# naver/dust3r

Hardware: NVIDIA H100
Metric: image-pairs/sec (512x384, ViT-L/B+DPT) (higher is better)
Workload: dtype bf16

## Files before the change

### dust3r_b200/csrc/d3r_common.cuh

```cuda
#pragma once
#include <cuda.h>
#include <cuda_runtime.h>
#include <cuda_bf16.h>
#include <cstdint>
#include <cstdio>
#include <cstdarg>

#include "../../include/dust3r_b200.h"

namespace d3r {

void set_error(const char* fmt, ...);

#define D3R_CHECK_ARG(cond, ...)                    \
  do {                                              \
    if (!(cond)) {                                  \
      ::d3r::set_error(__VA_ARGS__);                \
      return D3R_ERR_INVALID;                       \
    }                                               \
  } while (0)

#define D3R_CUDA(expr)                                                                     \
  do {                                                                                     \
    cudaError_t _e = (expr);                                                               \
    if (_e != cudaSuccess) {                                                               \
      ::d3r::set_error("%s failed: %s (%s:%d)", #expr, cudaGetErrorString(_e), __FILE__, __LINE__); \
      return D3R_ERR_CUDA;                                                                 \
    }                                                                                      \
  } while (0)

#define D3R_LAUNCH_CHECK()                                                                 \
  do {                                                                                     \
    cudaError_t _e = cudaGetLastError();                                                   \
    if (_e != cudaSuccess) {                                                               \
      ::d3r::set_error("kernel launch failed: %s (%s:%d)", cudaGetErrorString(_e), __FILE__, __LINE__); \
      return D3R_ERR_CUDA;                                                                 \
    }                                                                                      \
  } while (0)

__device__ __forceinline__ float warp_sum(float v) {
  v += __shfl_xor_sync(0xffffffffu, v, 16);
  v += __shfl_xor_sync(0xffffffffu, v, 8);
  v += __shfl_xor_sync(0xffffffffu, v, 4);
  v += __shfl_xor_sync(0xffffffffu, v, 2);
  v += __shfl_xor_sync(0xffffffffu, v, 1);
  return v;
}

__device__ __forceinline__ uint32_t pack_bf16x2(float a, float b) {
  __nv_bfloat162 h = __floats2bfloat162_rn(a, b);
  return *reinterpret_cast<uint32_t*>(&h);
}
__device__ __forceinline__ float2 bf16x2_to_float2(uint32_t w) {
  const __nv_bfloat162 h = *reinterpret_cast<const __nv_bfloat162*>(&w);
  return make_float2(__low2float(h), __high2float(h));
}

template <class ConfIn>
__device__ __forceinline__ void postprocess_pixel(float x, float y, float z, ConfIn conf_in, float* pts3d, float* conf, long long pix,
                                                  int depth_mode, int conf_mode, float cmin, float cmax) {
  float ox = x, oy = y, oz = z;
  if (depth_mode != 0) {
    const float d = sqrtf(x * x + y * y + z * z);
    const float dc = fmaxf(d, 1e-8f);
    const float s = (depth_mode == 2) ? expm1f(d) : d * d;
    ox = x / dc * s; oy = y / dc * s; oz = z / dc * s;
  }
  float* o = pts3d + pix * 3;
  o[0] = ox; o[1] = oy; o[2] = oz;
  if (conf_mode != 0) {
    const float c = conf_in();
    float r;
    if (conf_mode == 1) r = cmin + fminf(expf(c), cmax - cmin);
    else r = (cmax - cmin) * (1.f / (1.f + expf(-c))) + cmin;
    conf[pix] = r;
  }
}

int num_sms();

int encode_tensor_map(CUtensorMap* m, const void* base, int rank, const cuuint64_t* dims, const cuuint64_t* strides_bytes,
                      const cuuint32_t* box, const char* op, CUtensorMapDataType dtype = CU_TENSOR_MAP_DATA_TYPE_BFLOAT16);

inline bool first_launch_on_this_device(unsigned long long& mask) {
  int dev = 0;
  cudaGetDevice(&dev);
  const unsigned long long bit = 1ull << (dev & 63);
  if (mask & bit) return false;
  mask |= bit;
  return true;
}

}
```

### dust3r_b200/csrc/gemm_host.cu

```cuda
#include "gemm_wgmma.cuh"
#include "gemm_host.h"
#include "prof.h"

namespace d3r {
namespace gemm {

static int pick_block_n(int N, int mode, uint32_t flags, int conv_m_tiles = 0) {
  if (flags & F_HEAD_FINAL) return 128;
  if (conv_m_tiles > 0) return (N == 256 && (conv_m_tiles + 1) / 2 >= 4 * (num_sms() / 2)) ? 256 : 128;
  if (N % 256 == 0 && pick_epi(mode, flags) != EPI_GENERIC) return 256;
  if (N % 128 == 0) return 128;
  if (N % 64 == 0) return 64;
  return (N > 128) ? 128 : 64;
}

static int g_impl = 2;
static int g_pair_min_kb = 4;
static bool use_pair(int bn, int num_kb) { return bn >= 128 && (g_impl == 1 || (g_impl == 2 && num_kb >= g_pair_min_kb)); }

static int g_store = 1;
static int g_conv_store = 1;

static int grid_for(bool pair, int m_tiles, int n_tiles) {
  if (pair) {
    const int items = ((m_tiles + 1) / 2) * n_tiles;
    const int max_clusters = num_sms() / 2;
    return 2 * (items < max_clusters ? items : max_clusters);
  }
  const int items = m_tiles * n_tiles;
  return items < num_sms() ? items : num_sms();
}

static const char* prof_tag(const Params& p, int bn, bool pair) {
  return (p.mode == 1) ? ((p.flags & F_HEAD_FINAL) ? (pair ? "conv3x3_head_tail_2cta" : "conv3x3_head_tail")
                                                   : (pair ? "conv3x3_wgmma_2cta" : "conv3x3_wgmma"))
                       : (bn == 256 ? (pair ? "gemm_wgmma_2cta_bn256" : "gemm_wgmma_bn256")
                                    : (pair ? "gemm_wgmma_2cta_bn128" : (bn == 128 ? "gemm_wgmma_bn128" : "gemm_wgmma_bn64")));
}

template <int BN, int EPI, bool PAIR, bool TMA_STORE = false>
static int launch(const CUtensorMap& ta, const CUtensorMap& tb, const CUtensorMap& to, const Params& p, int m_tiles, int n_tiles,
                  cudaStream_t st) {
  constexpr int kSmem = Cfg<BN, TMA_STORE>::kSmemBytes;
  static unsigned long long attr_devices = 0;
  if (first_launch_on_this_device(attr_devices))
    D3R_CUDA(cudaFuncSetAttribute(gemm_kernel<BN, EPI, PAIR, TMA_STORE>, cudaFuncAttributeMaxDynamicSharedMemorySize, kSmem));
  const int grid = grid_for(PAIR, m_tiles, n_tiles);
  char detail[96];
  snprintf(detail, sizeof(detail), "M=%d N=%d K=%d flags=0x%x mode=%d epi=%d", p.M, p.N, p.K, (unsigned)p.flags, p.mode, EPI);
  prof::Scope scope(prof_tag(p, BN, PAIR), st, 2.0 * double(p.M) * double(p.N) * double(p.K), 0.0, 1, detail);
  D3R_CUDA(pdl::launch_clustered(gemm_kernel<BN, EPI, PAIR, TMA_STORE>, dim3(grid), dim3(kNumThreads), size_t(kSmem), st, PAIR ? 2 : 1,
                                 ta, tb, to, p));
  D3R_LAUNCH_CHECK();
  return D3R_OK;
}

template <int BN, bool PAIR>
static int launch_conv(const CUtensorMap& ta, const CUtensorMap& tb, const CUtensorMap& to, const ConvMaps& cm, const Params& p,
                       int m_tiles, int n_tiles, cudaStream_t st) {
  constexpr int kSmem = Cfg<BN, true>::kSmemBytes;
  static unsigned long long attr_devices = 0;
  if (first_launch_on_this_device(attr_devices))
    D3R_CUDA(cudaFuncSetAttribute(conv_kernel<BN, PAIR>, cudaFuncAttributeMaxDynamicSharedMemorySize, kSmem));
  const int grid = grid_for(PAIR, m_tiles, n_tiles);
  char detail[96];
  snprintf(detail, sizeof(detail), "M=%d N=%d K=%d flags=0x%x mode=%d epi=%d", p.M, p.N, p.K, (unsigned)p.flags, p.mode, EPI_GENERIC);
  prof::Scope scope(prof_tag(p, BN, PAIR), st, 2.0 * double(p.M) * double(p.N) * double(p.K), 0.0, 1, detail);
  D3R_CUDA(pdl::launch_clustered(conv_kernel<BN, PAIR>, dim3(grid), dim3(kNumThreads), size_t(kSmem), st, PAIR ? 2 : 1, ta, tb, to, cm, p));
  D3R_LAUNCH_CHECK();
  return D3R_OK;
}

template <int BN, bool PAIR>
static int dispatch_epi(int epi, const CUtensorMap& ta, const CUtensorMap& tb, const CUtensorMap* to, const Params& p, int m_tiles,
                        int n_tiles, cudaStream_t st) {
  if constexpr (BN == 256) {
    if (to) {
      switch (epi) {
        case EPI_RESID: return launch<BN, EPI_RESID, PAIR, true>(ta, tb, *to, p, m_tiles, n_tiles, st);
        case EPI_ACT: return launch<BN, EPI_ACT, PAIR, true>(ta, tb, *to, p, m_tiles, n_tiles, st);
        case EPI_ROPE: return launch<BN, EPI_ROPE, PAIR, true>(ta, tb, *to, p, m_tiles, n_tiles, st);
      }
    }
  }
  switch (epi) {
    case EPI_RESID: return launch<BN, EPI_RESID, PAIR>(ta, tb, tb, p, m_tiles, n_tiles, st);
    case EPI_ACT: return launch<BN, EPI_ACT, PAIR>(ta, tb, tb, p, m_tiles, n_tiles, st);
    case EPI_ROPE: return launch<BN, EPI_ROPE, PAIR>(ta, tb, tb, p, m_tiles, n_tiles, st);
  }
  if constexpr (BN == 128) return launch<128, EPI_GENERIC, PAIR>(ta, tb, tb, p, m_tiles, n_tiles, st);
  set_error("no BLOCK_N %d kernel for the generic epilogue", BN);
  return D3R_ERR_INVALID;
}

static int dispatch(int bn, const CUtensorMap& ta, const CUtensorMap& tb, const CUtensorMap* to, const Params& p, int m_tiles,
                    cudaStream_t st) {
  const int n_tiles = (p.N + bn - 1) / bn;
  const int epi = (bn >= 128) ? pick_epi(p.mode, p.flags) : EPI_GENERIC;
  const bool pair = use_pair(bn, p.num_kb);
  switch (bn) {
    case 256: return pair ? dispatch_epi<256, true>(epi, ta, tb, to, p, m_tiles, n_tiles, st) : dispatch_epi<256, false>(epi, ta, tb, to, p, m_tiles, n_tiles, st);
    case 128: return pair ? dispatch_epi<128, true>(epi, ta, tb, nullptr, p, m_tiles, n_tiles, st) : dispatch_epi<128, false>(epi, ta, tb, nullptr, p, m_tiles, n_tiles, st);
    case 64: return launch<64, EPI_GENERIC, false>(ta, tb, tb, p, m_tiles, n_tiles, st);
  }
  set_error("unsupported BLOCK_N %d", bn);
  return D3R_ERR_INVALID;
}

static int make_tmap_b(CUtensorMap* m, const void* B, int N, int taps, int Kc, int bn, int num_kb, const char* op) {
  cuuint64_t dims[3] = {(cuuint64_t)Kc, (cuuint64_t)taps, (cuuint64_t)N};
  cuuint64_t str[2] = {(cuuint64_t)Kc * 2, (cuuint64_t)taps * Kc * 2};
  cuuint32_t box[3] = {(cuuint32_t)BLOCK_K, 1, (cuuint32_t)(use_pair(bn, num_kb) ? bn / 2 : bn)};
  return encode_tensor_map(m, B, 3, dims, str, box, op);
}

int gemm_bf16(const void* A, long long lda, const void* B, Params p, cudaStream_t st) {
  D3R_CHECK_ARG(A && B, "gemm: null operand");
  D3R_CHECK_ARG(p.M > 0 && p.N > 0 && p.K > 0, "gemm: bad shape %d %d %d", p.M, p.N, p.K);
  D3R_CHECK_ARG(p.N % 32 == 0, "gemm: N=%d must be a multiple of 32", p.N);
  D3R_CHECK_ARG(p.K % 8 == 0 && lda % 8 == 0, "gemm: K=%d / lda=%lld must be multiples of 8 (16-byte TMA strides)", p.K, lda);
  D3R_CHECK_ARG((reinterpret_cast<uintptr_t>(A) & 15) == 0 && (reinterpret_cast<uintptr_t>(B) & 15) == 0, "gemm: operands must be 16-byte aligned");
// ... 17 lines not shown
                      (reinterpret_cast<uintptr_t>(p.out) & 15) == 0;
  if (staged) {
    cuuint64_t dims[2] = {(cuuint64_t)p.N, (cuuint64_t)p.M};
    cuuint64_t str[1] = {(cuuint64_t)row_bytes};
    cuuint32_t box[2] = {(cuuint32_t)(f32 ? 32 : 64), 64};
    rc = encode_tensor_map(&to, p.out, 2, dims, str, box, "gemm output", f32 ? CU_TENSOR_MAP_DATA_TYPE_FLOAT32 : CU_TENSOR_MAP_DATA_TYPE_BFLOAT16);
    if (rc) return rc;
  }
  return dispatch(bn, ta, tb, staged ? &to : nullptr, p, (p.M + BLOCK_M - 1) / BLOCK_M, st);
}

static int make_tmap_conv_io(CUtensorMap* m, const void* base, int B, int H, int W, int C, int tile_w, const char* op) {
  const int bw = tile_w < 64 ? tile_w : 64;
  cuuint64_t dims[4] = {(cuuint64_t)C, (cuuint64_t)W, (cuuint64_t)H, (cuuint64_t)B};
  cuuint64_t str[3] = {(cuuint64_t)C * 2, (cuuint64_t)W * C * 2, (cuuint64_t)H * W * C * 2};
  cuuint32_t box[4] = {64, (cuuint32_t)bw, (cuuint32_t)(64 / bw), 1};
  return encode_tensor_map(m, base, 4, dims, str, box, op);
}

static bool aligned16(const void* ptr) { return (reinterpret_cast<uintptr_t>(ptr) & 15) == 0; }

int conv3x3_bf16(const void* x_nhwc, const void* w_packed, int B, int H, int W, int Cin, int Cout, Params p, cudaStream_t st) {
  D3R_CHECK_ARG(x_nhwc && w_packed, "conv3x3: null operand");
  D3R_CHECK_ARG(Cin % 8 == 0 && Cout % 32 == 0, "conv3x3: Cin=%d must be a multiple of 8 and Cout=%d of 32", Cin, Cout);
  p.mode = 1;
  p.M = B * H * W;
  p.N = Cout;
  p.cin_blocks = (Cin + BLOCK_K - 1) / BLOCK_K;
  p.K = 9 * Cin;
  p.num_kb = 9 * p.cin_blocks;
  p.cB = B; p.cH = H; p.cW = W;
  int tw = 16;
  while (tw < W && tw < 128) tw *= 2;
  p.tile_w = tw;
  p.tile_h = BLOCK_M / tw;
  p.tiles_x = (W + p.tile_w - 1) / p.tile_w;
  p.tiles_y = (H + p.tile_h - 1) / p.tile_h;
  p.ldo = Cout;
  const int m_tiles = B * p.tiles_x * p.tiles_y;
  const bool staged = g_conv_store == 1 && (Cout == 256 || Cout == 128) && (p.flags & ~EpiMask<EPI_CONV>::value) == 0 &&
                      aligned16(p.out) && (!(p.flags & F_OUT2_RELU) || aligned16(p.out2)) && (!(p.flags & F_ADD0) || aligned16(p.add0)) &&
                      (!(p.flags & F_ADD1) || aligned16(p.add1));
  const int bn = pick_block_n(p.N, p.mode, p.flags, staged ? m_tiles : 0);
  CUtensorMap ta, tb;
  {
    cuuint64_t dims[4] = {(cuuint64_t)Cin, (cuuint64_t)W, (cuuint64_t)H, (cuuint64_t)B};
    cuuint64_t str[3] = {(cuuint64_t)Cin * 2, (cuuint64_t)W * Cin * 2, (cuuint64_t)H * W * Cin * 2};
    cuuint32_t box[4] = {(cuuint32_t)BLOCK_K, (cuuint32_t)p.tile_w, (cuuint32_t)p.tile_h, 1};
    int rc = encode_tensor_map(&ta, x_nhwc, 4, dims, str, box, "conv3x3");
    if (rc) return rc;
  }
  int rc = make_tmap_b(&tb, w_packed, Cout, 9, Cin, bn, p.num_kb, "conv3x3");
  if (rc) return rc;
  if (!staged) return dispatch(bn, ta, tb, nullptr, p, m_tiles, st);
  CUtensorMap to;
  ConvMaps cm;
  rc = make_tmap_conv_io(&to, p.out, B, H, W, Cout, p.tile_w, "conv3x3 output");
  if (rc) return rc;
  cm.out2 = cm.add0 = cm.add1 = to;
  const struct { uint32_t flag; const void* base; CUtensorMap* map; const char* op; } io[3] = {
      {F_OUT2_RELU, p.out2, &cm.out2, "conv3x3 out2"}, {F_ADD0, p.add0, &cm.add0, "conv3x3 add0"}, {F_ADD1, p.add1, &cm.add1, "conv3x3 add1"}};
  for (const auto& t : io) {
    if (!(p.flags & t.flag)) continue;
    rc = make_tmap_conv_io(t.map, t.base, B, H, W, Cout, p.tile_w, t.op);
    if (rc) return rc;
  }
  const int n_tiles = Cout / bn;
  const bool pair = use_pair(bn, p.num_kb);
  if (bn == 256) return pair ? launch_conv<256, true>(ta, tb, to, cm, p, m_tiles, n_tiles, st) : launch_conv<256, false>(ta, tb, to, cm, p, m_tiles, n_tiles, st);
  return pair ? launch_conv<128, true>(ta, tb, to, cm, p, m_tiles, n_tiles, st) : launch_conv<128, false>(ta, tb, to, cm, p, m_tiles, n_tiles, st);
}

int conv_transpose_bf16(const void* x_nhwc, const void* w_packed, void* out, const float* bias, int B, int h, int w, int Cin, int Cout,
                        int k, cudaStream_t st) {
  D3R_CHECK_ARG(x_nhwc && w_packed && out, "conv_transpose: null buffer");
  D3R_CHECK_ARG(B > 0 && h > 0 && w > 0 && Cin > 0 && Cout > 0 && k > 0, "conv_transpose: bad shape B=%d h=%d w=%d Cin=%d Cout=%d k=%d", B,
                h, w, Cin, Cout, k);
  D3R_CHECK_ARG(Cin % 8 == 0, "conv_transpose: Cin=%d must be a multiple of 8", Cin);
  D3R_CHECK_ARG(Cout % 2 == 0 && (k * k * Cout) % 32 == 0, "conv_transpose: Cout=%d must be even and k*k*Cout=%d a multiple of 32", Cout,
                k * k * Cout);
  Params p{};
  p.M = B * h * w; p.N = k * k * Cout; p.K = Cin;
  p.flags = F_CONVT | (bias ? F_BIAS : 0);
  p.out = out; p.bias = bias; p.ldo = 0;
  p.tk = k; p.th_in = h; p.tw_in = w; p.tCout = Cout;
  return gemm_bf16(x_nhwc, Cin, w_packed, p, st);
}

int conv3x3_head_tail(const void* x_nhwc, const void* w_packed, const float* bias, const float* w4, const float* b4, float* pts3d,
                      float* conf, int B, int H, int W, int depth_mode, int conf_mode, float conf_min, float conf_max, cudaStream_t st) {
  D3R_CHECK_ARG(x_nhwc && w_packed && w4 && b4 && pts3d, "conv3x3_head_tail: null buffer");
  D3R_CHECK_ARG(B > 0 && H > 0 && W > 0, "conv3x3_head_tail: bad shape B=%d H=%d W=%d", B, H, W);
  D3R_CHECK_ARG(depth_mode >= 0 && depth_mode <= 2, "conv3x3_head_tail: depth_mode %d out of range", depth_mode);
  D3R_CHECK_ARG(conf_mode >= 0 && conf_mode <= 2, "conv3x3_head_tail: conf_mode %d out of range", conf_mode);
  D3R_CHECK_ARG(conf_mode == 0 || conf, "conv3x3_head_tail: conf_mode %d without a conf buffer", conf_mode);
  Params p{};
  p.flags = F_HEAD_FINAL | (bias ? F_BIAS : 0);
  p.bias = bias;
  p.w4 = w4; p.b4 = b4;
  p.pts3d = pts3d; p.conf = conf;
  p.depth_mode = depth_mode; p.conf_mode = conf_mode;
  p.conf_min = conf_min; p.conf_max = conf_max;
  return conv3x3_bf16(x_nhwc, w_packed, B, H, W, 128, 128, p, st);
}

}
// ... 46 lines not shown
```

### dust3r_b200/csrc/gemm_wgmma.cuh

```cuda
#pragma once
#include "d3r_common.cuh"
#include "sm90_ptx.cuh"
#include "pdl.cuh"

namespace d3r {
namespace gemm {

constexpr int BLOCK_M = 128;
constexpr int BLOCK_K = 64;
constexpr int WGMMA_K = 16;
constexpr int kNumThreads = 384;
constexpr int kConsumerWarps = 8;

enum : uint32_t {
  F_BIAS = 1u << 0,
  F_GELU = 1u << 1,
  F_RELU = 1u << 2,
  F_OUT_F32 = 1u << 3,
  F_RESID_INPLACE = 1u << 4,
  F_ADD0 = 1u << 5,
  F_ADD1 = 1u << 6,
  F_OUT2_RELU = 1u << 7,
  F_ROPE = 1u << 8,
  F_CONVT = 1u << 9,
  F_HEAD_FINAL = 1u << 10,
  F_OUT2_BF16 = 1u << 11,
};

struct Params {
  int M, N, K;
  int num_kb;
  int mode;
  uint32_t flags;
  void* out;
  void* out2;
  const void* add0;
  const void* add1;
  const float* bias;
  long long ldo;
  const float* rope_cos;
  const float* rope_sin;
  int rope_cols, tokens_per_img, grid_w;
  int cB, cH, cW, cin_blocks, tile_w, tile_h, tiles_x, tiles_y;
  int tk, th_in, tw_in, tCout;
  const float* w4;
  const float* b4;
  float* pts3d;
  float* conf;
  int depth_mode;
  int conf_mode;
  float conf_min, conf_max;
};

enum : int { EPI_GENERIC = 0, EPI_RESID = 1, EPI_ACT = 2, EPI_ROPE = 3, EPI_CONV = 4 };
template <int EPI> struct EpiMask { static constexpr uint32_t value = 0xFFFFFFFFu; };
template <> struct EpiMask<EPI_RESID> { static constexpr uint32_t value = F_BIAS | F_RESID_INPLACE; };
template <> struct EpiMask<EPI_ACT> { static constexpr uint32_t value = F_BIAS | F_GELU | F_RELU; };
template <> struct EpiMask<EPI_ROPE> { static constexpr uint32_t value = F_BIAS | F_ROPE; };
template <> struct EpiMask<EPI_CONV> { static constexpr uint32_t value = F_BIAS | F_RELU | F_ADD0 | F_ADD1 | F_OUT2_RELU; };

struct ConvMaps {
  CUtensorMap out2, add0, add1;
};

__host__ __device__ inline int pick_epi(int mode, uint32_t flags) {
  if (mode != 0) return EPI_GENERIC;
  if ((flags & ~F_BIAS) == F_RESID_INPLACE) return EPI_RESID;
  if ((flags & ~EpiMask<EPI_ACT>::value) == 0) return EPI_ACT;
  if ((flags & ~EpiMask<EPI_ROPE>::value) == 0) return EPI_ROPE;
  return EPI_GENERIC;
}

template <int BLOCK_N, bool TMA_STORE = false>
struct Cfg {
  static constexpr int kStageA = BLOCK_M * BLOCK_K * 2;
  static constexpr int kStageB = BLOCK_N * BLOCK_K * 2;
  static constexpr int kStages = (BLOCK_N == 256) ? 4 : (BLOCK_N == 128) ? 6 : 8;
  static constexpr int kRing = kStages * (kStageA + kStageB);
  static constexpr int kOutBuf = 64 * 128;
  static constexpr int kStaging = TMA_STORE ? 2 * 2 * kOutBuf : 0;
  static constexpr int kSmemBytes = kRing + kStaging + 1024  + 256  + (TMA_STORE ? 0 : (4 * 128 + 16) * 4) ;
  static_assert(kSmemBytes <= 227 * 1024, "shared memory of one CTA");
};

__device__ __forceinline__ float gelu_erf(float x) {
  constexpr float kU = 0.84932180028801904f;
  constexpr float kP = 0.3275911f * 0.70710678118654752f / kU;
  const float u = fabsf(x) * kU;
  const float t = ptx::rcp_approx(fmaf(kP, u, 1.f));
  float poly = fmaf(0.5f * 1.061405429f, t, 0.5f * -1.453152027f);
  poly = fmaf(poly, t, 0.5f * 1.421413741f);
  poly = fmaf(poly, t, 0.5f * -0.284496736f);
  poly = fmaf(poly, t, 0.5f * 0.254829592f);
  const float e = ptx::ex2_approx(-u * u);
  const float h = x * (poly * t * e);
  return fmaxf(x, 0.f) - fabsf(h);
}

template <int BLOCK_N, int EPI, bool PAIR, bool TMA_STORE>
__device__ __forceinline__ void gemm_body(const CUtensorMap& tmap_a, const CUtensorMap& tmap_b, const CUtensorMap& tmap_o,
                                          const ConvMaps* cm, const Params& p) {
  static_assert(EPI == EPI_CONV ? (TMA_STORE && (BLOCK_N == 256 || BLOCK_N == 128))
                                : (!TMA_STORE || (BLOCK_N == 256 && EPI != EPI_GENERIC)),
                "TMA-store epilogue: specialised projection epilogues on 128x256 tiles, the conv epilogue on 128x256 / 128x128");
  using C = Cfg<BLOCK_N, TMA_STORE>;
  extern __shared__ uint8_t smem_raw[];
  uint8_t* smem = reinterpret_cast<uint8_t*>((reinterpret_cast<uintptr_t>(smem_raw) + 1023) & ~uintptr_t(1023));
  uint8_t* smem_a = smem;
  uint8_t* smem_b = smem + C::kStages * C::kStageA;
  uint8_t* smem_o = smem + C::kRing;
  uint64_t* bars = reinterpret_cast<uint64_t*>(smem + C::kRing + C::kStaging);
  uint64_t* full_bar = bars;
  uint64_t* empty_bar = bars + C::kStages;
  uint64_t* add_bar = bars + 2 * C::kStages;
  float* s_w4 = reinterpret_cast<float*>(reinterpret_cast<uint8_t*>(bars) + 256);

  const int warp = threadIdx.x >> 5, lane = threadIdx.x & 31;
  const uint32_t rank = PAIR ? ptx::cluster_ctarank() : 0u;
  const int n_tiles = (p.N + BLOCK_N - 1) / BLOCK_N;
  const int m_tiles = (p.mode == 1) ? p.cB * p.tiles_y * p.tiles_x : (p.M + BLOCK_M - 1) / BLOCK_M;
  const int m_groups = PAIR ? (m_tiles + 1) / 2 : m_tiles;
  const int total_items = m_groups * n_tiles;
  const int first_item = PAIR ? blockIdx.x / 2 : blockIdx.x;
  const int item_stride = PAIR ? gridDim.x / 2 : gridDim.x;

  if (threadIdx.x == 0) {
    ptx::prefetch_tmap(&tmap_a);
    ptx::prefetch_tmap(&tmap_b);
    if constexpr (TMA_STORE) ptx::prefetch_tmap(&tmap_o);
    for (int s = 0; s < C::kStages; ++s) {
      ptx::mbar_init(ptx::smem_u32(&full_bar[s]), 1);
      ptx::mbar_init(ptx::smem_u32(&empty_bar[s]), (PAIR ? 2 : 1) * kConsumerWarps);
    }
    if constexpr (EPI == EPI_CONV) {
      ptx::prefetch_tmap(&cm->out2);
      ptx::prefetch_tmap(&cm->add0);
      ptx::prefetch_tmap(&cm->add1);
      ptx::mbar_init(ptx::smem_u32(&add_bar[0]), 1);
      ptx::mbar_init(ptx::smem_u32(&add_bar[1]), 1);
    }
    ptx::fence_barrier_init();
  }
  if (!TMA_STORE && (p.flags & F_HEAD_FINAL) && threadIdx.x >= 128) {
    for (int i = threadIdx.x - 128; i < 4 * 128 + 4; i += 256) s_w4[i] = (i < 512) ? p.w4[i] : p.b4[i - 512];
  }
  __syncthreads();
  if constexpr (PAIR) ptx::cluster_sync();
  pdl::sync_with_predecessor();

  if (warp < 4) {
    ptx::setmaxnreg_dec<40>();
    if (warp == 0 && ptx::elect_one()) {
      int stage = 0;
      uint32_t phase = 0;
      for (int item = first_item; item < total_items; item += item_stride) {
        const int tn = item % n_tiles, tm = (item / n_tiles) * (PAIR ? 2 : 1) + int(rank);
        int cb = 0, cy0 = 0, cx0 = 0;
        if (p.mode == 1) {
          cb = tm / (p.tiles_y * p.tiles_x);
          const int r = tm - cb * (p.tiles_y * p.tiles_x);
          cy0 = (r / p.tiles_x) * p.tile_h;
          cx0 = (r % p.tiles_x) * p.tile_w;
        }
        for (int kb = 0; kb < p.num_kb; ++kb) {
          ptx::mbar_wait(ptx::smem_u32(&empty_bar[stage]), phase ^ 1);
          const uint32_t fb = ptx::smem_u32(&full_bar[stage]);
          ptx::mbar_arrive_expect_tx(fb, C::kStageA + C::kStageB);
          const uint32_t sa = ptx::smem_u32(smem_a + stage * C::kStageA);
          const uint32_t sb = ptx::smem_u32(smem_b + stage * C::kStageB);
          int ka, kt = 0;
          if (p.mode == 1) {
            const int tap = kb / p.cin_blocks, cblk = kb - tap * p.cin_blocks;
            const int dy = tap / 3, dx = tap - dy * 3;
            ptx::tma_load_4d(sa, &tmap_a, fb, cblk * BLOCK_K, cx0 + dx - 1, cy0 + dy - 1, cb);
            ka = cblk * BLOCK_K;
            kt = tap;
          } else {
            ptx::tma_load_2d(sa, &tmap_a, fb, kb * BLOCK_K, tm * BLOCK_M);
            ka = kb * BLOCK_K;
          }
          if constexpr (PAIR) {
            constexpr int kHalf = BLOCK_N / 2;
            ptx::tma_load_3d_mc(sb + rank * (kHalf * BLOCK_K * 2), &tmap_b, fb, ka, kt, tn * BLOCK_N + int(rank) * kHalf, 0x3);
          } else {
            ptx::tma_load_3d(sb, &tmap_b, fb, ka, kt, tn * BLOCK_N);
          }
          if (++stage == C::kStages) { stage = 0; phase ^= 1; }
        }
      }
    }
  } else {
    ptx::setmaxnreg_inc<232>();
    const int wg = (threadIdx.x >> 7) - 1;
    const int wq = warp & 3;
    const int q = lane & 3;
    const uint32_t flags = p.flags & EpiMask<EPI>::value;
    constexpr int kNB = BLOCK_N / 8;
    float acc[BLOCK_N / 2];
    int stage = 0;
    uint32_t phase = 0;
    uint32_t out_chunk = 0;
    auto release = [&](int s) {
      if (lane == 0) {
        if constexpr (PAIR) {
          ptx::mbar_arrive_cluster(ptx::smem_u32(&empty_bar[s]), 0);
          ptx::mbar_arrive_cluster(ptx::smem_u32(&empty_bar[s]), 1);
        } else {
          ptx::mbar_arrive(ptx::smem_u32(&empty_bar[s]));
        }
      }
    };
    const bool conv_issuer = EPI == EPI_CONV && (threadIdx.x & 127) == 0;
    const bool conv_two = EPI == EPI_CONV && (flags & (F_OUT2_RELU | F_ADD1)) != 0;
    const bool conv_add = EPI == EPI_CONV && (flags & (F_ADD0 | F_ADD1)) != 0;
    uint32_t add_phase = 0;
    auto conv_box = [&](int tm, int& bx, int& by, int& bb) {
      bb = tm / (p.tiles_y * p.tiles_x);
      const int r = tm - bb * (p.tiles_y * p.tiles_x);
      bx = (r % p.tiles_x) * p.tile_w + (64 * wg) % p.tile_w;
      by = (r / p.tiles_x) * p.tile_h + (64 * wg) / p.tile_w;
    };
    auto out_buf = [&](int i) { return ptx::smem_u32(smem_o + (wg * 2 + i) * C::kOutBuf); };
    auto issue_addends = [&](int tm, int ch) {
      int bx, by, bb;
      conv_box(tm, bx, by, bb);
      const uint32_t b0 = conv_two ? out_buf(0) : out_buf(out_chunk & 1);
      if (conv_two) ptx::bulk_wait_group_read<0>();
      else ptx::bulk_wait_group_read<1>();
      const uint32_t bar = ptx::smem_u32(&add_bar[wg]);
      ptx::mbar_arrive_expect_tx(bar, uint32_t(C::kOutBuf) * (((flags & F_ADD0) ? 1u : 0u) + ((flags & F_ADD1) ? 1u : 0u)));
      if (flags & F_ADD0) ptx::tma_load_4d(b0, &cm->add0, bar, ch, bx, by, bb);
      if (flags & F_ADD1) ptx::tma_load_4d(out_buf(1), &cm->add1, bar, ch, bx, by, bb);
    };
    for (int item = first_item; item < total_items; item += item_stride) {
      const int tn = item % n_tiles, tm = (item / n_tiles) * (PAIR ? 2 : 1) + int(rank);
      if constexpr (EPI == EPI_CONV) {
        if (conv_add && conv_issuer) issue_addends(tm, tn * BLOCK_N);
      }
      int prev = -1;
      for (int kb = 0; kb < p.num_kb; ++kb) {
        ptx::mbar_wait(ptx::smem_u32(&full_bar[stage]), phase);
        const uint64_t da = ptx::desc_kmajor_sw128(ptx::smem_u32(smem_a + stage * C::kStageA + wg * 64 * 128));
        const uint64_t db = ptx::desc_kmajor_sw128(ptx::smem_u32(smem_b + stage * C::kStageB));
        ptx::wgmma_fence();
#pragma unroll
        for (int k = 0; k < BLOCK_K / WGMMA_K; ++k) {
          if constexpr (BLOCK_N == 256) ptx::wgmma_m64n256k16_ss(acc, da + uint64_t(2 * k), db + uint64_t(2 * k), (kb | k) != 0 ? 1u : 0u);
          else if constexpr (BLOCK_N == 128) ptx::wgmma_m64n128k16_ss(acc, da + uint64_t(2 * k), db + uint64_t(2 * k), (kb | k) != 0 ? 1u : 0u);
          else ptx::wgmma_m64n64k16_ss(acc, da + uint64_t(2 * k), db + uint64_t(2 * k), (kb | k) != 0 ? 1u : 0u);
        }
        ptx::wgmma_commit();
        ptx::wgmma_wait<1>();
        if (prev >= 0) release(prev);
        prev = stage;
        if (++stage == C::kStages) { stage = 0; phase ^= 1; }
      }
      ptx::wgmma_wait<0>();
      ptx::reg_fence(acc);
      release(prev);

      bool valid[2];
      long long row_off[2];
      int tok[2] = {0, 0};
      long long pix[2] = {0, 0};
      int ct_b[2] = {0, 0}, ct_iy[2] = {0, 0}, ct_ix[2] = {0, 0};
#pragma unroll
      for (int h = 0; h < 2; ++h) {
        const int row_in_tile = wg * 64 + wq * 16 + (lane >> 2) + 8 * h;
        if (p.mode == 1) {
          const int cb = tm / (p.tiles_y * p.tiles_x);
          const int r = tm - cb * (p.tiles_y * p.tiles_x);
          const int y = (r / p.tiles_x) * p.tile_h + row_in_tile / p.tile_w;
          const int x = (r % p.tiles_x) * p.tile_w + row_in_tile % p.tile_w;
          valid[h] = (tm < m_tiles) && (y < p.cH) && (x < p.cW);
          pix[h] = (long long)(cb * p.cH + y) * p.cW + x;
          row_off[h] = pix[h] * p.ldo;
        } else {
          const int row = tm * BLOCK_M + row_in_tile;
          valid[h] = row < p.M;
          row_off[h] = (long long)row * p.ldo;
          if (flags & F_ROPE) tok[h] = row % p.tokens_per_img;
          if (flags & F_CONVT) {
            ct_b[h] = row / (p.th_in * p.tw_in);
            const int r = row - ct_b[h] * (p.th_in * p.tw_in);
            ct_iy[h] = r / p.tw_in;
            ct_ix[h] = r - ct_iy[h] * p.tw_in;
// ... 167 lines not shown
          if (flags & F_CONVT) {
            const int kk = col / p.tCout, co = col - kk * p.tCout;
            const int ky = kk / p.tk, kx = kk - ky * p.tk;
            off = ((long long)(ct_b[h] * p.th_in * p.tk + ct_iy[h] * p.tk + ky) * (p.tw_in * p.tk) + ct_ix[h] * p.tk + kx) * p.tCout + co;
          } else {
            off = row_off[h] + col;
          }
          if (flags & F_ADD0) {
            const float2 a = bf16x2_to_float2(__ldg(reinterpret_cast<const unsigned int*>(reinterpret_cast<const __nv_bfloat16*>(p.add0) + off)));
            v0 += a.x; v1 += a.y;
          }
          if (flags & F_ADD1) {
            const float2 a = bf16x2_to_float2(__ldg(reinterpret_cast<const unsigned int*>(reinterpret_cast<const __nv_bfloat16*>(p.add1) + off)));
            v0 += a.x; v1 += a.y;
          }
          if (flags & F_RELU) { v0 = fmaxf(v0, 0.f); v1 = fmaxf(v1, 0.f); }
          if (flags & (F_OUT_F32 | F_RESID_INPLACE)) {
            float2* o = reinterpret_cast<float2*>(reinterpret_cast<float*>(p.out) + off);
            if (flags & F_RESID_INPLACE) {
              const float2 r = *o;
              v0 += r.x; v1 += r.y;
            }
            *o = make_float2(v0, v1);
            if (flags & F_OUT2_BF16) *reinterpret_cast<uint32_t*>(reinterpret_cast<__nv_bfloat16*>(p.out2) + off) = pack_bf16x2(v0, v1);
          } else {
            *reinterpret_cast<uint32_t*>(reinterpret_cast<__nv_bfloat16*>(p.out) + off) = pack_bf16x2(v0, v1);
            if (flags & F_OUT2_RELU)
              *reinterpret_cast<uint32_t*>(reinterpret_cast<__nv_bfloat16*>(p.out2) + off) = pack_bf16x2(fmaxf(v0, 0.f), fmaxf(v1, 0.f));
          }
        }
      }
    }
    if constexpr (TMA_STORE) {
      if ((threadIdx.x & 127) == 0) ptx::bulk_wait_group<0>();
    }
  }
  if constexpr (PAIR) ptx::cluster_sync();
}

template <int BLOCK_N, int EPI, bool PAIR, bool TMA_STORE>
__global__ void __launch_bounds__(kNumThreads, 1)
gemm_kernel(const __grid_constant__ CUtensorMap tmap_a, const __grid_constant__ CUtensorMap tmap_b,
            const __grid_constant__ CUtensorMap tmap_o, const Params p) {
  gemm_body<BLOCK_N, EPI, PAIR, TMA_STORE>(tmap_a, tmap_b, tmap_o, nullptr, p);
}

template <int BLOCK_N, bool PAIR>
__global__ void __launch_bounds__(kNumThreads, 1)
conv_kernel(const __grid_constant__ CUtensorMap tmap_a, const __grid_constant__ CUtensorMap tmap_b,
            const __grid_constant__ CUtensorMap tmap_o, const __grid_constant__ ConvMaps cm, const Params p) {
  gemm_body<BLOCK_N, EPI_CONV, PAIR, true>(tmap_a, tmap_b, tmap_o, &cm, p);
}

}
}
```

### dust3r_b200/csrc/sm90_ptx.cuh

```cuda
#pragma once
#include <cuda.h>
#include <cuda_runtime.h>
#include <cuda_bf16.h>
#include <cstdint>

namespace d3r {
namespace ptx {

__device__ __forceinline__ uint32_t smem_u32(const void* p) { return static_cast<uint32_t>(__cvta_generic_to_shared(p)); }

__device__ __forceinline__ bool elect_one() {
  uint32_t pred = 0;
  asm volatile(
      "{\n"
      ".reg .b32 %%rx;\n"
      ".reg .pred %%px;\n"
      "elect.sync %%rx|%%px, %1;\n"
      "@%%px mov.s32 %0, 1;\n"
      "}\n"
      : "+r"(pred)
      : "r"(0xffffffffu));
  return pred != 0;
}

// ... 51 lines not shown

__device__ __forceinline__ void prefetch_tmap(const void* tmap) {
  asm volatile("prefetch.tensormap [%0];" ::"l"(reinterpret_cast<uint64_t>(tmap)) : "memory");
}
__device__ __forceinline__ void tma_load_2d(uint32_t dst, const void* tmap, uint32_t bar, int c0, int c1) {
  asm volatile(
      "cp.async.bulk.tensor.2d.shared::cluster.global.mbarrier::complete_tx::bytes [%0], [%1, {%3, %4}], [%2];"
      ::"r"(dst), "l"(reinterpret_cast<uint64_t>(tmap)), "r"(bar), "r"(c0), "r"(c1)
      : "memory");
}
__device__ __forceinline__ void tma_load_3d(uint32_t dst, const void* tmap, uint32_t bar, int c0, int c1, int c2) {
  asm volatile(
      "cp.async.bulk.tensor.3d.shared::cluster.global.mbarrier::complete_tx::bytes [%0], [%1, {%3, %4, %5}], [%2];"
      ::"r"(dst), "l"(reinterpret_cast<uint64_t>(tmap)), "r"(bar), "r"(c0), "r"(c1), "r"(c2)
      : "memory");
}
__device__ __forceinline__ void tma_load_4d(uint32_t dst, const void* tmap, uint32_t bar, int c0, int c1, int c2, int c3) {
  asm volatile(
      "cp.async.bulk.tensor.4d.shared::cluster.global.mbarrier::complete_tx::bytes [%0], [%1, {%3, %4, %5, %6}], [%2];"
      ::"r"(dst), "l"(reinterpret_cast<uint64_t>(tmap)), "r"(bar), "r"(c0), "r"(c1), "r"(c2), "r"(c3)
      : "memory");
}
__device__ __forceinline__ void tma_load_3d_mc(uint32_t dst, const void* tmap, uint32_t bar, int c0, int c1, int c2, uint16_t mask) {
  asm volatile(
      "cp.async.bulk.tensor.3d.shared::cluster.global.mbarrier::complete_tx::bytes.multicast::cluster [%0], [%1, {%3, %4, %5}], [%2], %6;"
      ::"r"(dst), "l"(reinterpret_cast<uint64_t>(tmap)), "r"(bar), "r"(c0), "r"(c1), "r"(c2), "h"(mask)
      : "memory");
}

__device__ __forceinline__ void tma_store_2d(const void* tmap, uint32_t src, int c0, int c1) {
  asm volatile("cp.async.bulk.tensor.2d.global.shared::cta.tile.bulk_group [%0, {%2, %3}], [%1];"
               ::"l"(reinterpret_cast<uint64_t>(tmap)), "r"(src), "r"(c0), "r"(c1) : "memory");
}
__device__ __forceinline__ void tma_store_4d(const void* tmap, uint32_t src, int c0, int c1, int c2, int c3) {
  asm volatile("cp.async.bulk.tensor.4d.global.shared::cta.tile.bulk_group [%0, {%2, %3, %4, %5}], [%1];"
               ::"l"(reinterpret_cast<uint64_t>(tmap)), "r"(src), "r"(c0), "r"(c1), "r"(c2), "r"(c3) : "memory");
}
__device__ __forceinline__ void tma_reduce_add_2d(const void* tmap, uint32_t src, int c0, int c1) {
  asm volatile("cp.reduce.async.bulk.tensor.2d.global.shared::cta.add.tile.bulk_group [%0, {%2, %3}], [%1];"
               ::"l"(reinterpret_cast<uint64_t>(tmap)), "r"(src), "r"(c0), "r"(c1) : "memory");
}
__device__ __forceinline__ void bulk_commit_group() { asm volatile("cp.async.bulk.commit_group;" ::: "memory"); }
template <int N> __device__ __forceinline__ void bulk_wait_group_read() { asm volatile("cp.async.bulk.wait_group.read %0;" ::"n"(N) : "memory"); }
template <int N> __device__ __forceinline__ void bulk_wait_group() { asm volatile("cp.async.bulk.wait_group %0;" ::"n"(N) : "memory"); }
__device__ __forceinline__ void st_shared_b32(uint32_t addr, uint32_t v) { asm volatile("st.shared.b32 [%0], %1;" ::"r"(addr), "r"(v) : "memory"); }
__device__ __forceinline__ uint32_t ld_shared_b32(uint32_t addr) {
  uint32_t v;
  asm volatile("ld.shared.b32 %0, [%1];" : "=r"(v) : "r"(addr) : "memory");
  return v;
}
__device__ __forceinline__ void st_shared_v2_f32(uint32_t addr, float a, float b) {
  asm volatile("st.shared.v2.f32 [%0], {%1, %2};" ::"r"(addr), "f"(a), "f"(b) : "memory");
}
__device__ __forceinline__ void named_bar_sync(uint32_t id, uint32_t count) { asm volatile("bar.sync %0, %1;" ::"r"(id), "r"(count) : "memory"); }

__device__ __forceinline__ uint32_t cluster_ctarank() {
  uint32_t r;
  asm volatile("mov.u32 %0, %%cluster_ctarank;" : "=r"(r));
  return r;
}
__device__ __forceinline__ void cluster_sync() {
  asm volatile("barrier.cluster.arrive.release.aligned;\nbarrier.cluster.wait.acquire.aligned;" ::: "memory");
}
__device__ __forceinline__ void mbar_arrive_cluster(uint32_t bar, uint32_t rank) {
  asm volatile(
      "{\n"
      ".reg .b32 raddr;\n"
      "mapa.shared::cluster.u32 raddr, %0, %1;\n"
      "mbarrier.arrive.shared::cluster.b64 _, [raddr];\n"
      "}\n" ::"r"(bar), "r"(rank) : "memory");
}

__device__ __forceinline__ float ex2_approx(float x) { float y; asm("ex2.approx.ftz.f32 %0, %1;" : "=f"(y) : "f"(x)); return y; }
__device__ __forceinline__ float rcp_approx(float x) { float y; asm("rcp.approx.ftz.f32 %0, %1;" : "=f"(y) : "f"(x)); return y; }
__device__ __forceinline__ float rsqrt_approx(float x) { float y; asm("rsqrt.approx.ftz.f32 %0, %1;" : "=f"(y) : "f"(x)); return y; }
__device__ __forceinline__ float sqrt_approx(float x) { float y; asm("sqrt.approx.ftz.f32 %0, %1;" : "=f"(y) : "f"(x)); return y; }

template <int N> __device__ __forceinline__ void setmaxnreg_dec() { asm volatile("setmaxnreg.dec.sync.aligned.u32 %0;" ::"n"(N)); }
template <int N> __device__ __forceinline__ void setmaxnreg_inc() { asm volatile("setmaxnreg.inc.sync.aligned.u32 %0;" ::"n"(N)); }

__device__ __forceinline__ void wgmma_fence() { asm volatile("wgmma.fence.sync.aligned;" ::: "memory"); }
__device__ __forceinline__ void wgmma_commit() { asm volatile("wgmma.commit_group.sync.aligned;" ::: "memory"); }
template <int N> __device__ __forceinline__ void wgmma_wait() { asm volatile("wgmma.wait_group.sync.aligned %0;" ::"n"(N) : "memory"); }
template <int N> __device__ __forceinline__ void reg_fence(float (&d)[N]) {
#pragma unroll
  for (int i = 0; i < N; ++i) asm volatile("" : "+f"(d[i])::"memory");
}

__device__ __forceinline__ uint64_t desc_sw128(uint32_t smem_addr, uint32_t lbo_bytes) {
  uint64_t d = 0;
  d |= uint64_t((smem_addr & 0x3FFFF) >> 4);
  d |= uint64_t(lbo_bytes >> 4) << 16;
  d |= uint64_t(1024 >> 4) << 32;
  d |= uint64_t(1) << 62;
  return d;
}
__device__ __forceinline__ uint64_t desc_kmajor_sw128(uint32_t smem_addr) { return desc_sw128(smem_addr, 16); }
__device__ __forceinline__ uint64_t desc_mnmajor_sw128(uint32_t smem_addr) { return desc_sw128(smem_addr, 1024); }

__device__ __forceinline__ void wgmma_m64n64k16_ss(float* d, uint64_t desc_a, uint64_t desc_b, uint32_t accumulate) {
  asm volatile(
      "{\n"
      ".reg .pred p;\n"
      "setp.ne.b32 p, %34, 0;\n"
      "wgmma.mma_async.sync.aligned.m64n64k16.f32.bf16.bf16 "
      "{%0, %1, %2, %3, %4, %5, %6, %7, %8, %9, %10, %11, %12, %13, %14, %15, %16, %17, %18, %19, %20, %21, %22, %23, %24, %25, %26, %27, %28, %29, %30, %31}, %32, %33, p, 1, 1, 0, 0;\n"
// ... 52 lines not shown
```

Baseline: 233.2.

## Add dedicated DPT head-tail conv kernel with double-buffered accumulators and epilogue overlap

Adds a specialised head_tail_kernel for the final 3x3 conv plus the 1x1 head projection. It keeps two accumulator sets so the WGMMA mainloop of the next tile is issued while the current tile's fused ReLU/projection/postprocess epilogue runs. Bias and transposed w4 are staged in shared memory and read with vector loads. This is meant to hide epilogue latency in the head conv, at the cost of doubled accumulator registers and a larger static unrolled schedule.

After: 236.3 (median of 6 runs). +1.3%, better.

```diff
diff --git a/dust3r_b200/csrc/d3r_common.cuh b/dust3r_b200/csrc/d3r_common.cuh
--- a/dust3r_b200/csrc/d3r_common.cuh
+++ b/dust3r_b200/csrc/d3r_common.cuh
@@ -56,9 +56,7 @@
   return make_float2(__low2float(h), __high2float(h));
 }
 
-template <class ConfIn>
-__device__ __forceinline__ void postprocess_pixel(float x, float y, float z, ConfIn conf_in, float* pts3d, float* conf, long long pix,
-                                                  int depth_mode, int conf_mode, float cmin, float cmax) {
+__device__ __forceinline__ void postprocess_pts(float x, float y, float z, float* pts3d, long long pix, int depth_mode) {
   float ox = x, oy = y, oz = z;
   if (depth_mode != 0) {
     const float d = sqrtf(x * x + y * y + z * z);
@@ -68,13 +66,16 @@
   }
   float* o = pts3d + pix * 3;
   o[0] = ox; o[1] = oy; o[2] = oz;
-  if (conf_mode != 0) {
-    const float c = conf_in();
-    float r;
-    if (conf_mode == 1) r = cmin + fminf(expf(c), cmax - cmin);
-    else r = (cmax - cmin) * (1.f / (1.f + expf(-c))) + cmin;
-    conf[pix] = r;
-  }
+}
+__device__ __forceinline__ float postprocess_conf(float c, int conf_mode, float cmin, float cmax) {
+  if (conf_mode == 1) return cmin + fminf(expf(c), cmax - cmin);
+  return (cmax - cmin) * (1.f / (1.f + expf(-c))) + cmin;
+}
+template <class ConfIn>
+__device__ __forceinline__ void postprocess_pixel(float x, float y, float z, ConfIn conf_in, float* pts3d, float* conf, long long pix,
+                                                  int depth_mode, int conf_mode, float cmin, float cmax) {
+  postprocess_pts(x, y, z, pts3d, pix, depth_mode);
+  if (conf_mode != 0) conf[pix] = postprocess_conf(conf_in(), conf_mode, cmin, cmax);
 }
 
 int num_sms();
diff --git a/dust3r_b200/csrc/gemm_host.cu b/dust3r_b200/csrc/gemm_host.cu
--- a/dust3r_b200/csrc/gemm_host.cu
+++ b/dust3r_b200/csrc/gemm_host.cu
@@ -67,6 +67,21 @@
   snprintf(detail, sizeof(detail), "M=%d N=%d K=%d flags=0x%x mode=%d epi=%d", p.M, p.N, p.K, (unsigned)p.flags, p.mode, EPI_GENERIC);
   prof::Scope scope(prof_tag(p, BN, PAIR), st, 2.0 * double(p.M) * double(p.N) * double(p.K), 0.0, 1, detail);
   D3R_CUDA(pdl::launch_clustered(conv_kernel<BN, PAIR>, dim3(grid), dim3(kNumThreads), size_t(kSmem), st, PAIR ? 2 : 1, ta, tb, to, cm, p));
+  D3R_LAUNCH_CHECK();
+  return D3R_OK;
+}
+
+template <bool PAIR>
+static int launch_head(const CUtensorMap& ta, const CUtensorMap& tb, const Params& p, int m_tiles, cudaStream_t st) {
+  constexpr int kSmem = Cfg<128>::kSmemBytes;
+  static unsigned long long attr_devices = 0;
+  if (first_launch_on_this_device(attr_devices))
+    D3R_CUDA(cudaFuncSetAttribute(head_tail_kernel<PAIR>, cudaFuncAttributeMaxDynamicSharedMemorySize, kSmem));
+  const int grid = grid_for(PAIR, m_tiles, 1);
+  char detail[96];
+  snprintf(detail, sizeof(detail), "M=%d N=%d K=%d flags=0x%x mode=%d epi=%d", p.M, p.N, p.K, (unsigned)p.flags, p.mode, EPI_GENERIC);
+  prof::Scope scope(prof_tag(p, 128, PAIR), st, 2.0 * double(p.M) * double(p.N) * double(p.K), 0.0, 1, detail);
+  D3R_CUDA(pdl::launch_clustered(head_tail_kernel<PAIR>, dim3(grid), dim3(kNumThreads), size_t(kSmem), st, PAIR ? 2 : 1, ta, tb, p));
   D3R_LAUNCH_CHECK();
   return D3R_OK;
 }
@@ -190,6 +205,11 @@
   }
   int rc = make_tmap_b(&tb, w_packed, Cout, 9, Cin, bn, p.num_kb, "conv3x3");
   if (rc) return rc;
+  if ((p.flags & F_HEAD_FINAL) && g_conv_store == 1) {
+    D3R_CHECK_ARG(Cin == 128 && Cout == 128 && (p.flags & ~EpiMask<EPI_HEAD>::value) == 0, "conv3x3: head tail with Cin=%d Cout=%d flags=0x%x",
+                  Cin, Cout, (unsigned)p.flags);
+    return use_pair(bn, p.num_kb) ? launch_head<true>(ta, tb, p, m_tiles, st) : launch_head<false>(ta, tb, p, m_tiles, st);
+  }
   if (!staged) return dispatch(bn, ta, tb, nullptr, p, m_tiles, st);
   CUtensorMap to;
   ConvMaps cm;
diff --git a/dust3r_b200/csrc/gemm_wgmma.cuh b/dust3r_b200/csrc/gemm_wgmma.cuh
--- a/dust3r_b200/csrc/gemm_wgmma.cuh
+++ b/dust3r_b200/csrc/gemm_wgmma.cuh
@@ -52,12 +52,13 @@
   float conf_min, conf_max;
 };
 
-enum : int { EPI_GENERIC = 0, EPI_RESID = 1, EPI_ACT = 2, EPI_ROPE = 3, EPI_CONV = 4 };
+enum : int { EPI_GENERIC = 0, EPI_RESID = 1, EPI_ACT = 2, EPI_ROPE = 3, EPI_CONV = 4, EPI_HEAD = 5 };
 template <int EPI> struct EpiMask { static constexpr uint32_t value = 0xFFFFFFFFu; };
 template <> struct EpiMask<EPI_RESID> { static constexpr uint32_t value = F_BIAS | F_RESID_INPLACE; };
 template <> struct EpiMask<EPI_ACT> { static constexpr uint32_t value = F_BIAS | F_GELU | F_RELU; };
 template <> struct EpiMask<EPI_ROPE> { static constexpr uint32_t value = F_BIAS | F_ROPE; };
 template <> struct EpiMask<EPI_CONV> { static constexpr uint32_t value = F_BIAS | F_RELU | F_ADD0 | F_ADD1 | F_OUT2_RELU; };
+template <> struct EpiMask<EPI_HEAD> { static constexpr uint32_t value = F_BIAS | F_HEAD_FINAL; };
 
 struct ConvMaps {
   CUtensorMap out2, add0, add1;
@@ -79,7 +80,7 @@
   static constexpr int kRing = kStages * (kStageA + kStageB);
   static constexpr int kOutBuf = 64 * 128;
   static constexpr int kStaging = TMA_STORE ? 2 * 2 * kOutBuf : 0;
-  static constexpr int kSmemBytes = kRing + kStaging + 1024  + 256  + (TMA_STORE ? 0 : (4 * 128 + 16) * 4) ;
+  static constexpr int kSmemBytes = kRing + kStaging + 1024  + 256  + (TMA_STORE ? 0 : (4 * 128 + 4 + 128) * 4) ;
   static_assert(kSmemBytes <= 227 * 1024, "shared memory of one CTA");
 };
 
@@ -100,9 +101,11 @@
 template <int BLOCK_N, int EPI, bool PAIR, bool TMA_STORE>
 __device__ __forceinline__ void gemm_body(const CUtensorMap& tmap_a, const CUtensorMap& tmap_b, const CUtensorMap& tmap_o,
                                           const ConvMaps* cm, const Params& p) {
-  static_assert(EPI == EPI_CONV ? (TMA_STORE && (BLOCK_N == 256 || BLOCK_N == 128))
-                                : (!TMA_STORE || (BLOCK_N == 256 && EPI != EPI_GENERIC)),
-                "TMA-store epilogue: specialised projection epilogues on 128x256 tiles, the conv epilogue on 128x256 / 128x128");
+  static_assert(EPI == EPI_CONV   ? (TMA_STORE && (BLOCK_N == 256 || BLOCK_N == 128))
+                : EPI == EPI_HEAD ? (!TMA_STORE && BLOCK_N == 128)
+                                  : (!TMA_STORE || (BLOCK_N == 256 && EPI != EPI_GENERIC)),
+                "TMA-store epilogue: specialised projection epilogues on 128x256 tiles, the conv epilogue on 128x256 / 128x128; "
+                "the head tail on 128x128 with register stores");
   using C = Cfg<BLOCK_N, TMA_STORE>;
   extern __shared__ uint8_t smem_raw[];
   uint8_t* smem = reinterpret_cast<uint8_t*>((reinterpret_cast<uintptr_t>(smem_raw) + 1023) & ~uintptr_t(1023));
@@ -114,6 +117,7 @@
   uint64_t* empty_bar = bars + C::kStages;
   uint64_t* add_bar = bars + 2 * C::kStages;
   float* s_w4 = reinterpret_cast<float*>(reinterpret_cast<uint8_t*>(bars) + 256);
+  float* s_bias = s_w4 + 4 * 128 + 4;
 
   const int warp = threadIdx.x >> 5, lane = threadIdx.x & 31;
   const uint32_t rank = PAIR ? ptx::cluster_ctarank() : 0u;
@@ -141,7 +145,12 @@
     }
     ptx::fence_barrier_init();
   }
-  if (!TMA_STORE && (p.flags & F_HEAD_FINAL) && threadIdx.x >= 128) {
+  if constexpr (EPI == EPI_HEAD) {
+    if (threadIdx.x >= 128) {
+      for (int i = threadIdx.x - 128; i < 4 * 128 + 4 + 128; i += 256)
+        s_w4[i] = (i < 512) ? p.w4[(i & 3) * 128 + (i >> 2)] : (i < 516) ? p.b4[i - 512] : (p.flags & F_BIAS) ? p.bias[i - 516] : 0.f;
+    }
+  } else if (!TMA_STORE && (p.flags & F_HEAD_FINAL) && threadIdx.x >= 128) {
     for (int i = threadIdx.x - 128; i < 4 * 128 + 4; i += 256) s_w4[i] = (i < 512) ? p.w4[i] : p.b4[i - 512];
   }
   __syncthreads();
@@ -232,6 +241,121 @@
       if (flags & F_ADD0) ptx::tma_load_4d(b0, &cm->add0, bar, ch, bx, by, bb);
       if (flags & F_ADD1) ptx::tma_load_4d(out_buf(1), &cm->add1, bar, ch, bx, by, bb);
     };
+    if constexpr (EPI == EPI_HEAD) {
+      constexpr int kHeadAhead = 2;
+      float acc_a[BLOCK_N / 2], acc_b[BLOCK_N / 2];
+      int rel_stage = 0, pending = 0;
+      auto issue = [&](float (&a)[BLOCK_N / 2], int kb) {
+        ptx::mbar_wait(ptx::smem_u32(&full_bar[stage]), phase);
+        const uint64_t da = ptx::desc_kmajor_sw128(ptx::smem_u32(smem_a + stage * C::kStageA + wg * 64 * 128));
+        const uint64_t db = ptx::desc_kmajor_sw128(ptx::smem_u32(smem_b + stage * C::kStageB));
+        ptx::wgmma_fence();
+#pragma unroll
+        for (int k = 0; k < BLOCK_K / WGMMA_K; ++k)
+          ptx::wgmma_m64n128k16_ss(a, da + uint64_t(2 * k), db + uint64_t(2 * k), (kb | k) != 0 ? 1u : 0u);
+        ptx::wgmma_commit();
+        if (++stage == C::kStages) { stage = 0; phase ^= 1; }
+        ++pending;
+      };
+      auto retire = [&](auto keep) {
+        ptx::wgmma_wait<decltype(keep)::value>();
+        for (; pending > decltype(keep)::value; --pending) {
+          release(rel_stage);
+          if (++rel_stage == C::kStages) rel_stage = 0;
+        }
+      };
+      auto epilogue = [&](const float (&a)[BLOCK_N / 2], int tm) {
+        float head_acc[2][4] = {{0.f, 0.f, 0.f, 0.f}, {0.f, 0.f, 0.f, 0.f}};
+#pragma unroll
+        for (int j = 0; j < kNB; ++j) {
+          float2 b = make_float2(0.f, 0.f);
+          if (flags & F_BIAS) b = ptx::ld_shared_v2_f32(ptx::smem_u32(s_bias + 8 * j + 2 * q));
+#pragma unroll
+          for (int h = 0; h < 2; ++h)
+#pragma unroll
+            for (int e = 0; e < 2; ++e) {
+              float v = a[4 * j + 2 * h + e];
+              if (flags & F_BIAS) v += e ? b.y : b.x;
+              v = fmaxf(v, 0.f);
+              const float4 w = ptx::ld_shared_v4_f32(ptx::smem_u32(s_w4 + 4 * (8 * j + 2 * q + e)));
+              head_acc[h][0] += v * w.x;
+              head_acc[h][1] += v * w.y;
+              head_acc[h][2] += v * w.z;
+              head_acc[h][3] += v * w.w;
+            }
+        }
+#pragma unroll
+        for (int h = 0; h < 2; ++h)
+#pragma unroll
+          for (int o = 0; o < 4; ++o) {
+            head_acc[h][o] += __shfl_xor_sync(0xffffffffu, head_acc[h][o], 1);
+            head_acc[h][o] += __shfl_xor_sync(0xffffffffu, head_acc[h][o], 2);
+          }
+        const bool h1 = (q & 1) != 0;
+        const int cb = tm / (p.tiles_y * p.tiles_x);
+        const int r = tm - cb * (p.tiles_y * p.tiles_x);
+        const int row_in_tile = wg * 64 + wq * 16 + (lane >> 2) + (h1 ? 8 : 0);
+        const int y = (r / p.tiles_x) * p.tile_h + row_in_tile / p.tile_w;
+        const int x = (r % p.tiles_x) * p.tile_w + row_in_tile % p.tile_w;
+        if (tm < m_tiles && y < p.cH && x < p.cW) {
+          const long long px = (long long)(cb * p.cH + y) * p.cW + x;
+          const float4 b4 = ptx::ld_shared_v4_f32(ptx::smem_u32(s_w4 + 512));
+          if (q < 2) {
+            postprocess_pts((h1 ? head_acc[1][0] : head_acc[0][0]) + b4.x, (h1 ? head_acc[1][1] : head_acc[0][1]) + b4.y,
+                            (h1 ? head_acc[1][2] : head_acc[0][2]) + b4.z, p.pts3d, px, p.depth_mode);
+          } else if (p.conf_mode != 0) {
+            p.conf[px] = postprocess_conf((h1 ? head_acc[1][3] : head_acc[0][3]) + b4.w, p.conf_mode, p.conf_min, p.conf_max);
+          }
+        }
+      };
+      constexpr int kHeadKb = 9 * 128 / BLOCK_K;
+      auto rest = [&](float (&nxt)[BLOCK_N / 2]) {
+#pragma unroll
+        for (int kb = kHeadAhead; kb < kHeadKb; ++kb) {
+          issue(nxt, kb);
+          retire(std::integral_constant<int, 1>{});
+        }
+      };
+      auto ahead = [&](float (&nxt)[BLOCK_N / 2]) {
+#pragma unroll
+        for (int kb = 0; kb < kHeadAhead; ++kb) issue(nxt, kb);
+        retire(std::integral_constant<int, kHeadAhead>{});
+      };
+      auto tm_of = [&](int item) { return (item / n_tiles) * (PAIR ? 2 : 1) + int(rank); };
+      int item = first_item;
+      if (item < total_items) {
+#pragma unroll
+        for (int kb = 0; kb < kHeadKb; ++kb) {
+          issue(acc_a, kb);
+          retire(std::integral_constant<int, 1>{});
+        }
+        while (true) {
+          if (item + item_stride >= total_items) {
+            retire(std::integral_constant<int, 0>{});
+            ptx::reg_fence(acc_a);
+            epilogue(acc_a, tm_of(item));
+            break;
+          }
+          ahead(acc_b);
+          ptx::reg_fence(acc_a);
+          epilogue(acc_a, tm_of(item));
+          rest(acc_b);
+          item += item_stride;
+          if (item + item_stride >= total_items) {
+            retire(std::integral_constant<int, 0>{});
+            ptx::reg_fence(acc_b);
+            epilogue(acc_b, tm_of(item));
+            break;
+          }
+          ahead(acc_a);
+          ptx::reg_fence(acc_b);
+          epilogue(acc_b, tm_of(item));
+          rest(acc_a);
+          item += item_stride;
+        }
+      }
+    }
+    if constexpr (EPI != EPI_HEAD)
     for (int item = first_item; item < total_items; item += item_stride) {
       const int tn = item % n_tiles, tm = (item / n_tiles) * (PAIR ? 2 : 1) + int(rank);
       if constexpr (EPI == EPI_CONV) {
@@ -505,5 +629,11 @@
   gemm_body<BLOCK_N, EPI_CONV, PAIR, true>(tmap_a, tmap_b, tmap_o, &cm, p);
 }
 
-}
-}
+template <bool PAIR>
+__global__ void __launch_bounds__(kNumThreads, 1)
+head_tail_kernel(const __grid_constant__ CUtensorMap tmap_a, const __grid_constant__ CUtensorMap tmap_b, const Params p) {
+  gemm_body<128, EPI_HEAD, PAIR, false>(tmap_a, tmap_b, tmap_b, nullptr, p);
+}
+
+}
+}
diff --git a/dust3r_b200/csrc/sm90_ptx.cuh b/dust3r_b200/csrc/sm90_ptx.cuh
--- a/dust3r_b200/csrc/sm90_ptx.cuh
+++ b/dust3r_b200/csrc/sm90_ptx.cuh
@@ -127,6 +127,16 @@
 __device__ __forceinline__ void st_shared_v2_f32(uint32_t addr, float a, float b) {
   asm volatile("st.shared.v2.f32 [%0], {%1, %2};" ::"r"(addr), "f"(a), "f"(b) : "memory");
 }
+__device__ __forceinline__ float2 ld_shared_v2_f32(uint32_t addr) {
+  float2 v;
+  asm volatile("ld.shared.v2.f32 {%0, %1}, [%2];" : "=f"(v.x), "=f"(v.y) : "r"(addr) : "memory");
+  return v;
+}
+__device__ __forceinline__ float4 ld_shared_v4_f32(uint32_t addr) {
+  float4 v;
+  asm volatile("ld.shared.v4.f32 {%0, %1, %2, %3}, [%4];" : "=f"(v.x), "=f"(v.y), "=f"(v.z), "=f"(v.w) : "r"(addr) : "memory");
+  return v;
+}
 __device__ __forceinline__ void named_bar_sync(uint32_t id, uint32_t count) { asm volatile("bar.sync %0, %1;" ::"r"(id), "r"(count) : "memory"); }
 
 __device__ __forceinline__ uint32_t cluster_ctarank() {
```
